# NoelShin/zutis

Measured on AMD Instinct MI355X. Metric: images/sec, COCO2017-val-shaped ViT-B/16 dense semantic segmentation @336px (ZUTIS forward + semantic predict), batches of 32 per GPU, 3 independent batches in flight, higher is better.
Workload: dtype f16x3 (fp32-class)

## Files before the change

### include/zutis_hip.h

```cpp
#ifndef ZUTIS_HIP_H
#define ZUTIS_HIP_H

#include <stddef.h>

#ifdef __cplusplus
extern "C" {
#endif

typedef struct ihipStream_t* zh_stream_t;

#define ZH_OK 0
#define ZH_ERR_ARG (-1)
#define ZH_ERR_HIP (-2)
#define ZH_ERR_WORKSPACE (-3)

#define ZH_ACT_NONE 0
#define ZH_ACT_QUICKGELU 1
#define ZH_ACT_RELU 2
#define ZH_ACT_SIGMOID 3
#define ZH_ACT_GELU_ERF 4

#define ZH_ABI_VERSION 245
int zh_version(void);
const char* zh_arch(void);
const char* zh_last_error(void);

int zh_dev_set_gemm_overrides(int group_m, int tile, int tile_small);

int zh_dev_gemm_plan(int mode, int M, int N, int K, int batch, long lda, long ldw, long ldc, long strideC, long planeC,
                     long ldr, long strideR, int res_rows, int out_kind, int act, int flags,
                     const void* C, const void* bias, const void* residual, int has_pos, int* plan);

int zh_dev_set_gemm_persist(int workgroups);

int zh_gemm_f16(const void* A, long lda, long strideA, const void* W, long ldw, long strideW,
                void* C, long ldc, long strideC, int out_f16,
                const float* bias, const float* residual, long ldr, long strideR, int res_rows,
                const void* pos_y, const void* pos_x, long ld_pos, int pos_h, int pos_w, int pos_f16,
                int act, int M, int N, int K, int batch, zh_stream_t stream);

int zh_gemm_f16_res16(const void* A, long lda, long strideA, const void* W, long ldw, long strideW,
                      void* C, long ldc, long strideC,
                      const float* bias, const void* residual, long ldr, long strideR, int res_rows,
                      int M, int N, int K, int batch, zh_stream_t stream);

#define ZH_GEMM_FIXED_K_ORDER 1
int zh_gemm_f16x3(const void* A, long lda, long strideA, long planeA, const void* W, long ldw, long strideW, long planeW,
                  void* C, long ldc, long strideC, long planeC, int out_kind, float out_scale,
                  const float* bias, const float* residual, long ldr, long strideR, int res_rows,
                  const void* pos_y, const void* pos_x, long ld_pos, int pos_h, int pos_w, int pos_f16,
                  int act, int M, int N, int K, int batch, int flags, zh_stream_t stream);

#define ZH_ATTN_QUERY_BLOCK 128
#define ZH_ATTN_KEY_TILE_F16 64
#define ZH_ATTN_KEY_TILE_X3 32
size_t zh_attention_splitk_workspace_size(int batch, int heads, int Tq, int head_dim, int ksplit);
int zh_attention_f16_splitk(const void* Q, long ldq, long strideQ, const void* K, long ldk, long strideK,
                            const void* V, long ldv, long strideV, void* O, long ldo, long strideO,
                            int batch, int heads, int Tq, int Tk, int head_dim, float scale,
                            long planeQ, long planeK, long planeV, long planeO, int ksplit, void* workspace, size_t workspace_bytes,
                            zh_stream_t stream);
int zh_attention_f16(const void* Q, long ldq, long strideQ, const void* K, long ldk, long strideK,
                     const void* V, long ldv, long strideV, void* O, long ldo, long strideO,
                     int batch, int heads, int Tq, int Tk, int head_dim, float scale,
                     long planeQ, long planeK, long planeV, long planeO, zh_stream_t stream);

int zh_attention_causal_f16(const void* Q, long ldq, long strideQ, const void* K, long ldk, long strideK,
                            const void* V, long ldv, long strideV, void* O, long ldo, long strideO,
                            int batch, int heads, int T, int head_dim, float scale,
                            long planeQ, long planeK, long planeV, long planeO, zh_stream_t stream);

int zh_dev_attention_plan(const void* Q, long ldq, long strideQ, const void* K, long ldk, long strideK,
                          const void* V, long ldv, long strideV, const void* O, long ldo, long strideO,
                          int batch, int heads, int Tq, int Tk, int head_dim, int causal,
                          long planeQ, long planeK, long planeV, long planeO, int ksplit, const void* workspace, size_t workspace_bytes,
                          int* plan);

int zh_embed_tokens_f32(const long long* tokens, const float* table, const float* pos, float* out, long n, int ctx, int D,
                        int vocab, zh_stream_t stream);
int zh_eot_rows_f32(const long long* tokens, const float* x, float* out, long n, int ctx, int D, zh_stream_t stream);
int zh_group_mean_l2norm(const float* x, float* out, int groups, int T, int E, zh_stream_t stream);

int zh_layernorm_f32(const float* x, long in_group_rows, long in_group_stride, long in_offset,
                     long out_group_rows, long out_group_stride, long out_offset,
                     const float* gamma, const float* beta, float eps,
                     float* out_f32, void* out_f16, void* out_f16_plus, float* out_f32_plus,
                     const float* add, int add_rows, int rows, int D, long lo_plane, int* status, zh_stream_t stream);
int zh_layernorm_f16(const void* x, long in_group_rows, long in_group_stride, long in_offset,
                     long out_group_rows, long out_group_stride, long out_offset,
                     const float* gamma, const float* beta, float eps,
                     float* out_f32, void* out_f16, void* out_f16_plus, float* out_f32_plus,
                     const float* add, int add_rows, int rows, int D, long lo_plane, int* status, zh_stream_t stream);
#define ZH_STATUS_RANGE 1
#define ZH_STATUS_NONFINITE 2
#define ZH_STATUS_LABEL 4

int zh_sum_layernorm_f32(const float* parts, int n_parts, long part_stride, const float* bias, const float* residual,
                         float* out_sum, const float* gamma, const float* beta, float eps,
                         float* out_f32, void* out_f16, long lo_plane,
                         long out_group_rows, long out_group_stride, long out_offset, int skip_first_in_group,
                         const float* gamma2, const float* beta2, float eps2, float* out2_f32, void* out2_f16, long lo_plane2,
                         long out2_group_rows, long out2_group_stride, long out2_offset,
                         int rows, int D, int* status, zh_stream_t stream);

int zh_assemble_tokens_ln(const float* patch_emb, const float* class_embedding, const float* pos_embed,
                          const float* gamma, const float* beta, float eps, float* out,
                          int B, int T, int D, zh_stream_t stream);

int zh_assemble_tokens_ln_f16(const float* patch_emb, const float* class_embedding, const float* pos_embed,
                              const float* gamma, const float* beta, float eps, void* out,
                              int B, int T, int D, zh_stream_t stream);

int zh_l2norm_rows(const float* x, float* out_f32, void* out_f16, float eps, int rows, int D, long lo_plane, float f16_scale, zh_stream_t stream);

size_t zh_global_ln_l2_workspace_size(int B, int M, int C);
int zh_global_ln_l2(const float* x, float* out_f32, void* out_f16, float eps, float l2_eps,
                    int B, int M, int C, void* workspace, size_t workspace_bytes, long lo_plane, float f16_scale, int* status,
                    zh_stream_t stream);

int zh_im2col_f16(const float* x, void* out, int B, int Cin, int H, int W, int patch, int Kpad, int pad_to_patch,
                  long lo_plane, zh_stream_t stream);

int zh_posembed_bicubic(const float* pos, float* out, int grid, int h, int w, int D, float scale_h, float scale_w,
                        int has_cls, zh_stream_t stream);

int zh_upsample2x_bilinear_cl(const float* x, float* out_f32, void* out_f16, int B, int h, int w, int D, long lo_plane,
                              int relu, zh_stream_t stream);

int zh_sine_pe(float* out, int h, int w, int D, float temperature, zh_stream_t stream);

int zh_add_rowperiodic_f16(const void* a, const float* add, void* out, long rows, int D, int add_rows, long a_lo_plane,
                           long lo_plane, zh_stream_t stream);

int zh_fill_f32(float* x, float value, long n, zh_stream_t stream);

int zh_cast_f32_f16(const float* x, const float* add, int add_rows, void* out, long rows, int D, long lo_plane, float f16_scale,
                    zh_stream_t stream);

int zh_upsample_argmax(const float* logits_lo, long long* labels, int B, int n, int h, int w, int H, int W,
                       float scale_h, float scale_w, zh_stream_t stream);

#define ZH_GT_U8 0
#define ZH_GT_RG16 1
int zh_upsample_argmax_score(const float* logits_lo, const unsigned char* gt, int gt_format, long long* hist_accum,
                             long long* labels, int B, int n, int h, int w, int H, int W, float scale_h, float scale_w,
                             zh_stream_t stream);

int zh_upsample_argmax_bytes(const float* logits_lo, unsigned char* labels_out, int label_format, unsigned char* overlay_out,
                             const unsigned char* packed, const int* desc, const unsigned char* palette, int alpha,
                             int B, int n, int h, int w, int H, int W, float scale_h, float scale_w, zh_stream_t stream);

int zh_upsample_bilinear_nchw(const float* x, float* out, unsigned char* mask_u8, float threshold, long planes,
                              int h, int w, int H, int W, float scale_h, float scale_w, zh_stream_t stream);

int zh_select_upsample_mask(const float* objectness, const float* masks, unsigned char* out_u8, long long* index, int B, int Q,
                            int h, int w, int H, int W, float scale_h, float scale_w, float threshold, zh_stream_t stream);

int zh_resize_nearest_u8(const unsigned char* x, unsigned char* out, int h, int w, int H, int W, float scale_h, float scale_w,
                         zh_stream_t stream);

int zh_confusion_hist(const long long* label_true, const long long* label_pred, long long* hist_accum, long total,
                      int n_class, zh_stream_t stream);

int zh_instance_mask_stats(const float* mask_proposals, long stride_image, float threshold, int B, int Q, int M,
                           float* sizes, float* confidence, unsigned char* binary, int* range_flag, zh_stream_t stream);
size_t zh_masked_mean_workspace_size(int B, int Q, int M, int E);
int zh_masked_mean_tokens(const float* tokens, const unsigned char* binary, const float* sizes, float* avg,
                          int B, int Q, int M, int E, void* workspace, size_t workspace_bytes, zh_stream_t stream);
int zh_instance_classify(const float* avg, const float* text, const float* confidence, float temperature,
                         int rows, int n_classes, int E, long long* category, float* score, zh_stream_t stream);
size_t zh_mask_iou_workspace_size(int n, long pixels);
int zh_mask_iou_counts(const unsigned char* masks, int n, long pixels, int* inter, int* uni,
                       void* workspace, size_t workspace_bytes, zh_stream_t stream);

#define ZH_RCN_KMAX 152
int zh_resize_crop_normalize_u8(const unsigned char* packed, long packed_bytes, const int* desc, int B, int n_px, int kmax,
                                const float* lut, float* out, zh_stream_t stream);
#define ZH_FILTER_BILINEAR 2
#define ZH_FILTER_BICUBIC 3
int zh_resize_normalize_u8(const unsigned char* packed, long packed_bytes, const int* desc, int B, int out_h, int out_w, int filter,
                           int kmax, const float* lut, float* out, zh_stream_t stream);

int zh_denormalize_u8(const float* x, unsigned char* rgb, int H, int W, const float* mean3, const float* std3,
                      zh_stream_t stream);
int zh_bgrid_coords(const unsigned char* rgb, int H, int W, double sigma_spatial, double sigma_luma, double sigma_chroma,
                    int* coords, zh_stream_t stream);
// ... 173 lines not shown
```

### zutis_amd/csrc/capi.hip

```cpp
#include "common.h"
#include <stdarg.h>

static thread_local char g_err[512] = "";

void zh_set_error(const char* fmt, ...) {
  va_list ap;
  va_start(ap, fmt);
  vsnprintf(g_err, sizeof(g_err), fmt, ap);
  va_end(ap);
}

extern "C" const char* zh_last_error(void) { return g_err; }
extern "C" int zh_version(void) { return ZH_ABI_VERSION; }
extern "C" const char* zh_arch(void) { return "gfx950"; }

#include <stdlib.h>
#include "gemm_dispatch.h"
static GemmDevOverrides& gemm_dev_state() {
  static GemmDevOverrides o = [] {
    GemmDevOverrides v{4, 0, 0};
    if (const char* g = getenv("ZH_GEMM_GROUP_M")) { const int x = atoi(g); if (x >= 1) v.group_m = x; }
    if (const char* t = getenv("ZH_GEMM_TILE")) v.tile = atoi(t);
    if (const char* t = getenv("ZH_GEMM_TILE_SMALL")) v.tile_small = atoi(t);
    return v;
  }();
  return o;
}
const GemmDevOverrides& gemm_dev_overrides() { return gemm_dev_state(); }
extern "C" int zh_dev_set_gemm_overrides(int group_m, int tile, int tile_small) {
  ZH_CHECK_ARG(group_m >= 0 && tile >= 0 && tile_small >= 0, "zh_dev_set_gemm_overrides: negative argument");
  GemmDevOverrides& o = gemm_dev_state();
  o.group_m = group_m >= 1 ? group_m : 4;
  o.tile = tile;
  o.tile_small = tile_small;
  return ZH_OK;
}

extern "C" int zh_dev_gemm_plan(int mode, int M, int N, int K, int batch, long lda, long ldw, long ldc, long strideC, long planeC,
                                long ldr, long strideR, int res_rows, int out_kind, int act, int flags,
                                const void* C, const void* bias, const void* residual, int has_pos, int* plan) {
  ZH_CHECK_ARG(plan && mode >= GEMM_F16 && mode <= GEMM_X2, "zh_dev_gemm_plan: null plan or mode %d not in {0 f16, 1 res16, 2 x3, 3 x2}", mode);
  ZH_CHECK_ARG(M > 0 && N > 0 && K > 0 && batch > 0, "zh_dev_gemm_plan: bad shape M=%d N=%d K=%d batch=%d", M, N, K, batch);
  const GemmProblem q = {mode, M, N, K, batch, lda, ldw, ldc, strideC, planeC, ldr, strideR, res_rows, out_kind, act, flags,
                         (uintptr_t)C, (uintptr_t)bias, (uintptr_t)residual, has_pos != 0, mode == GEMM_RES16};
  GemmPlan g;
  const int rc = mode <= GEMM_RES16 ? gemm_plan_f16(q, gemm_dev_overrides(), &g) : gemm_plan_x3(q, gemm_dev_overrides(), &g);
  if (rc != ZH_OK) return rc;
  const GemmTile* t = gemm_plan_tile(mode, g.code);
  ZH_CHECK_ARG(t || g.family == GEMM_SKINNY, "zh_dev_gemm_plan: the plan's tile code %d has no table row", g.code);
  plan[0] = g.family; plan[1] = g.code; plan[2] = t ? gemm_tile_m(*t) : 32; plan[3] = t ? gemm_tile_n(*t) : 32;
  plan[4] = g.path; plan[5] = (int)g.peel_rows;
  return ZH_OK;
}

#include "attention_dispatch.h"
extern "C" int zh_dev_attention_plan(const void* Q, long ldq, long strideQ, const void* K, long ldk, long strideK,
                                     const void* V, long ldv, long strideV, const void* O, long ldo, long strideO,
                                     int batch, int heads, int Tq, int Tk, int head_dim, int causal,
                                     long planeQ, long planeK, long planeV, long planeO, int ksplit, const void* workspace, size_t workspace_bytes,
                                     int* plan) {
  ZH_CHECK_ARG(plan, "zh_dev_attention_plan: null plan");
  AttnPlan a;
  const int rc = attn_plan(attn_problem(Q, ldq, strideQ, K, ldk, strideK, V, ldv, strideV, O, ldo, strideO, batch, heads, Tq, Tk, head_dim, causal,
                                        planeQ, planeK, planeV, planeO, ksplit, workspace, workspace_bytes), &a);
  if (rc != ZH_OK) return rc;
  ZH_CHECK_ARG(a.workspace_bytes <= 0x7FFFFFFF, "zh_dev_attention_plan: a workspace of %zu bytes does not fit the int row", a.workspace_bytes);
  plan[0] = a.variant; plan[1] = a.key_tile; plan[2] = a.nqb; plan[3] = (int)a.items; plan[4] = (int)a.grid; plan[5] = a.pipe;
  plan[6] = a.ksplit; plan[7] = a.kchunk; plan[8] = (int)a.workspace_bytes; plan[9] = (int)a.combine_grid;
  return ZH_OK;
}

static int gemm_persist_valid(int n) { return n >= 0 && n % 8 == 0; }
static int g_gemm_persist = [] {
  const char* e = getenv("ZH_GEMM_PERSIST");
  if (!e) return -1;
  char* end = nullptr;
  const long v = strtol(e, &end, 10);
  if (end == e || *end != 0 || v < 0 || v > (1 << 20) || !gemm_persist_valid((int)v)) {
    fprintf(stderr, "zutis_hip: ZH_GEMM_PERSIST=%s ignored (not 0 or a multiple of 8)\n", e);
    return -1;
  }
  return (int)v;
}();
int gemm_persist_cus() {
  if (g_gemm_persist >= 0) return g_gemm_persist;
  static const int auto_cus = [] {
    int dev = 0, cus = 0;
    if (hipGetDevice(&dev) != hipSuccess || hipDeviceGetAttribute(&cus, hipDeviceAttributeMultiprocessorCount, dev) != hipSuccess || cus < 8) return 256;
    return cus / 8 * 8;
  }();
  return auto_cus;
}
extern "C" int zh_dev_set_gemm_persist(int workgroups) {
  ZH_CHECK_ARG(workgroups >= -1 && (workgroups == -1 || gemm_persist_valid(workgroups)), "zh_dev_set_gemm_persist: %d is not -1 (auto), 0 (off) or a multiple of 8", workgroups);
  g_gemm_persist = workgroups;
  return ZH_OK;
}
```

### zutis_amd/csrc/gemm.hip

```cpp
#include "gemm_kernel.h"
#include "gemm_dispatch.h"

template <int WM, int WN, int TM, int TN, int STAGES, int VEC>
static bool launch_gemm(const GemmArgs& p, int batch, int out_f16, int res_f16, hipStream_t stream) {
  const int key = res_f16 * 16 + out_f16 * 8 + p.act;
  switch (key) {
    case 0 + ZH_ACT_NONE: launch_one<WM, WN, TM, TN, STAGES, 0, ZH_ACT_NONE, VEC, 0>(p, batch, stream); return true;
    case 0 + ZH_ACT_SIGMOID: launch_one<WM, WN, TM, TN, STAGES, 0, ZH_ACT_SIGMOID, VEC, 0>(p, batch, stream); return true;
    case 8 + ZH_ACT_NONE: launch_one<WM, WN, TM, TN, STAGES, 1, ZH_ACT_NONE, VEC, 0>(p, batch, stream); return true;
    case 8 + ZH_ACT_QUICKGELU: launch_one<WM, WN, TM, TN, STAGES, 1, ZH_ACT_QUICKGELU, VEC, 0>(p, batch, stream); return true;
    case 8 + ZH_ACT_RELU: launch_one<WM, WN, TM, TN, STAGES, 1, ZH_ACT_RELU, VEC, 0>(p, batch, stream); return true;
    case 8 + ZH_ACT_GELU_ERF: launch_one<WM, WN, TM, TN, STAGES, 1, ZH_ACT_GELU_ERF, VEC, 0>(p, batch, stream); return true;
    case 16 + 8 + ZH_ACT_NONE: launch_one<WM, WN, TM, TN, STAGES, 3, ZH_ACT_NONE, VEC, 0>(p, batch, stream); return true;
    default: return false;
  }
}

static int gemm_f16_impl(const void* A, long lda, long strideA, const void* W, long ldw, long strideW,
                         void* C, long ldc, long strideC, int out_f16,
                         const float* bias, const void* residual, int res_f16, long ldr, long strideR, int res_rows,
                         const void* pos_y, const void* pos_x, long ld_pos, int pos_h, int pos_w, int pos_f16,
                         int act, int M, int N, int K, int batch, hipStream_t stream) {
  GemmArgs p;
  GemmProblem q;
  GemmPlan plan;
  int rc = gemm_prepare("zh_gemm_f16", res_f16 ? GEMM_RES16 : GEMM_F16, A, lda, strideA, 0, W, ldw, strideW, 0, C, ldc, strideC, 0, out_f16 ? 1 : 0, 1.0f,
                        bias, residual, ldr, strideR, res_rows, pos_y, pos_x, ld_pos, pos_h, pos_w, pos_f16, act, M, N, K, batch, 0, &p, &q);
  if (rc != ZH_OK) return rc;
  ZH_CHECK_ARG(!res_f16 || (out_f16 && act == ZH_ACT_NONE), "zh_gemm_f16_res16: an fp16 residual goes with an fp16 output and no activation");
  if ((rc = gemm_plan_f16(q, gemm_dev_overrides(), &plan)) != ZH_OK) return rc;
  if (plan.peel_rows)
    return gemm_tail_peel(plan.peel_rows, M, A, lda, C, ldc, out_f16 ? 2 : 4, residual, ldr, res_f16 ? 2 : 4, res_rows,
                          [&](const void* a, void* c, const void* r, int rows, int m) {
                            return gemm_f16_impl(a, lda, strideA, W, ldw, strideW, c, ldc, strideC, out_f16, bias, r, res_f16, ldr, strideR, rows,
                                                 pos_y, pos_x, ld_pos, pos_h, pos_w, pos_f16, act, m, N, K, 1, stream);
                          });
  const int ok = gemm_launch_plan<GEMM_TILES_F16>(plan, [&](auto row) {
    constexpr GemmTile t = decltype(row)::t;
    return launch_gemm<t.wm, t.wn, t.tm, t.tn, t.stages, decltype(row)::vec>(p, batch, out_f16, res_f16, stream);
  }, std::make_index_sequence<std::size(GEMM_TILES_F16)>{});
  ZH_CHECK_ARG(ok >= 0, "zh_gemm_f16: the plan's tile code %d has no table row", plan.code);
  ZH_CHECK_ARG(ok, "zh_gemm_f16: (out_f16=%d, act=%d) is not an instantiated epilogue (f32: none|sigmoid; f16: none|quickgelu|relu|gelu_erf)",
               out_f16, act);
  ZH_CHECK_LAUNCH("zh_gemm_f16");
  return ZH_OK;
}

extern "C" int zh_gemm_f16(const void* A, long lda, long strideA, const void* W, long ldw, long strideW,
                           void* C, long ldc, long strideC, int out_f16,
                           const float* bias, const float* residual, long ldr, long strideR, int res_rows,
                           const void* pos_y, const void* pos_x, long ld_pos, int pos_h, int pos_w, int pos_f16,
                           int act, int M, int N, int K, int batch, hipStream_t stream) {
  return gemm_f16_impl(A, lda, strideA, W, ldw, strideW, C, ldc, strideC, out_f16, bias, residual, 0, ldr, strideR, res_rows,
                       pos_y, pos_x, ld_pos, pos_h, pos_w, pos_f16, act, M, N, K, batch, stream);
}

extern "C" int zh_gemm_f16_res16(const void* A, long lda, long strideA, const void* W, long ldw, long strideW,
                                 void* C, long ldc, long strideC,
                                 const float* bias, const void* residual, long ldr, long strideR, int res_rows,
                                 int M, int N, int K, int batch, hipStream_t stream) {
  ZH_CHECK_ARG(residual, "zh_gemm_f16_res16: null residual (zh_gemm_f16 is the form without one)");
  return gemm_f16_impl(A, lda, strideA, W, ldw, strideW, C, ldc, strideC, 1, bias, residual, 1, ldr, strideR, res_rows,
                       nullptr, nullptr, 0, 0, 0, 0, ZH_ACT_NONE, M, N, K, batch, stream);
}
```

### zutis_amd/csrc/gemm_dispatch.h

```cpp
#pragma once
#include "common.h"
#include <utility>
#ifndef RING64
#define RING64 6
#endif
#ifndef ZH_SKINNY_MAX_ROWS
#define ZH_SKINNY_MAX_ROWS 128
#endif
#ifndef ZH_SKINNY_MAX_BLOCKS
#define ZH_SKINNY_MAX_BLOCKS 512
#endif

struct GemmDevOverrides { int group_m; int tile; int tile_small; };
const GemmDevOverrides& gemm_dev_overrides();

enum { GEMM_F16 = 0, GEMM_RES16 = 1, GEMM_X3 = 2, GEMM_X2 = 3 };
enum { GEMM_RING = 0, GEMM_SKINNY = 1 };
enum { GEMM_STORE_SCALAR = 0, GEMM_STORE_DIRECT = 1, GEMM_STORE_WIDE = 2 };

struct GemmProblem {
  int mode, M, N, K, batch; long lda, ldw, ldc, strideC, planeC, ldr, strideR; int res_rows, out_kind, act, flags;
  uintptr_t C, bias, residual; bool has_pos, res_f16;
};
struct GemmPlan { int family, code, path; long peel_rows; };

struct GemmTile { int code, wm, wn, tm, tn, stages; };
constexpr GemmTile GEMM_TILES_F16[] = {
  {128, 2, 2, 4, 4, 4},
  {64, 2, 2, 4, 2, 4},
  {192, 2, 4, 8, 3, 4},
  {256, 2, 4, 8, 4, 4},
  {2128, 2, 2, 4, 4, 8},
  {2064, 2, 2, 4, 2, 8},
  {3064, 2, 2, 2, 2, 8},
  {7032, 2, 2, 2, 2, 7},
  {7096, 2, 2, 4, 3, 5},
  {7128, 2, 2, 4, 4, 5},
};
constexpr GemmTile GEMM_TILES_X3[] = {
  {64, 2, 2, 4, 2, 3},
  {512, 2, 4, 8, 4, 2},
  {448, 2, 4, 6, 4, 2},
  {256, 4, 2, 4, 4, 3},
  {192, 4, 2, 3, 4, 3},
  {96, 4, 2, 2, 3, 3},
  {3064, 2, 2, 2, 2, 4},
  {3066, 2, 2, 2, 2, RING64},
  {1288, 4, 2, 2, 4, 4},
  {6496, 4, 2, 2, 3, 2},
  {6464, 4, 2, 2, 2, 3},
  {7096, 4, 2, 2, 3, 4},
  {7128, 4, 2, 2, 4, 3},
};
constexpr GemmTile GEMM_TILES_X2[] = {
  {64, 2, 2, 4, 2, 3},
  {512, 4, 2, 4, 8, 3},
  {5122, 2, 4, 8, 4, 2},
  {5124, 2, 4, 8, 4, 3},
  {4484, 4, 2, 3, 8, 3},
  {448, 2, 4, 6, 4, 3},
  {256, 4, 2, 4, 4, 3},
  {192, 4, 2, 3, 4, 4},
  {96, 4, 2, 2, 3, 3},
  {3064, 2, 2, 2, 2, 4},
  {3066, 2, 2, 2, 2, RING64},
  {6464, 4, 2, 2, 2, 3},
  {1288, 4, 2, 2, 4, 4},
  {6496, 4, 2, 2, 3, 2},
};
constexpr int gemm_tile_m(const GemmTile& t) { return t.wm * t.tm * 16; }
constexpr int gemm_tile_n(const GemmTile& t) { return t.wn * t.tn * 16; }
template <size_t R>
constexpr const GemmTile* gemm_tile(const GemmTile (&rows)[R], int code) {
  for (size_t i = 0; i < R; ++i) if (rows[i].code == code) return &rows[i];
  return nullptr;
}
static inline const GemmTile* gemm_plan_tile(int mode, int code) {
  if (mode <= GEMM_RES16) return code ? gemm_tile(GEMM_TILES_F16, code) : GEMM_TILES_F16;
  if (mode == GEMM_X3) return code ? gemm_tile(GEMM_TILES_X3, code) : GEMM_TILES_X3;
  return code ? gemm_tile(GEMM_TILES_X2, code) : GEMM_TILES_X2;
}
template <const auto& ROWS, size_t I, int VEC> struct GemmRow { static constexpr GemmTile t = ROWS[I]; static constexpr int vec = VEC; };
template <const auto& ROWS, class L, size_t... I>
static inline int gemm_launch_plan(const GemmPlan& plan, L&& launch, std::index_sequence<I...>) {
  if (plan.path != GEMM_STORE_WIDE) return plan.path == GEMM_STORE_SCALAR ? launch(GemmRow<ROWS, 0, 0>{}) : launch(GemmRow<ROWS, 0, 1>{});
  int ok = -1;
  (void)((ROWS[I].code == plan.code && ((ok = launch(GemmRow<ROWS, I, 2>{})), true)) || ...);
  return ok;
}

static inline bool gemm_vec_ok(const GemmProblem& q) {
  const int esz = q.out_kind == 0 ? 4 : 2;
  return q.N % 4 == 0 && q.ldc % 4 == 0 && q.strideC % 4 == 0 && (q.C & (4 * esz - 1)) == 0 && (!q.bias || (q.bias & 15) == 0) &&
         (!q.residual || (q.ldr % 4 == 0 && q.strideR % 4 == 0 && (q.residual & (q.res_f16 ? 7 : 15)) == 0));
}
static inline bool gemm_wide_ok(const GemmProblem& q) {
  const int esz = q.out_kind == 0 ? 4 : 2;
  if (!(gemm_vec_ok(q) && (q.C & 15) == 0 && (q.ldc * esz) % 16 == 0 && (q.strideC * esz) % 16 == 0 && (q.N * esz) % 16 == 0)) return false;
  if (q.mode <= GEMM_RES16)
    return !q.residual || (q.res_f16 ? (q.ldr % 8 == 0 && q.strideR % 8 == 0 && (q.residual & 15) == 0) : q.out_kind == 0);
  return (q.out_kind != 1 || !q.residual) && (q.out_kind != 2 || q.planeC % 8 == 0);
}

static inline bool zh_pos_tables_ok(const void* pos_y, const void* pos_x, long ld_pos, int pos_h, int pos_w, int N) {
  if (!pos_y && !pos_x) return true;
  return pos_y && pos_x && pos_h > 0 && pos_w > 0 && ld_pos >= N && ld_pos % 8 == 0 && N % 4 == 0 &&
         (((uintptr_t)pos_y | (uintptr_t)pos_x) & 15) == 0;
}

template <class Args>
static inline int gemm_prepare(const char* fn, int mode, const void* A, long lda, long strideA, long planeA, const void* W, long ldw, long strideW,
                               long planeW, void* C, long ldc, long strideC, long planeC, int out_kind, float out_scale, const float* bias,
                               const void* residual, long ldr, long strideR, int res_rows, const void* pos_y, const void* pos_x, long ld_pos,
                               int pos_h, int pos_w, int pos_f16, int act, int M, int N, int K, int batch, int flags, Args* pp, GemmProblem* q) {
  ZH_CHECK_ARG(A && W && C, "%s: null operand", fn);
  ZH_CHECK_ARG(M > 0 && N > 0 && K > 0 && batch > 0, "%s: bad shape M=%d N=%d K=%d batch=%d", fn, M, N, K, batch);
  ZH_CHECK_ARG(K % 64 == 0, "%s: K=%d must be a multiple of 64", fn, K);
  ZH_CHECK_ARG(lda % 8 == 0 && ldw % 8 == 0 && strideA % 8 == 0 && strideW % 8 == 0 && planeA % 8 == 0 && planeW % 8 == 0,
               "%s: lda/ldw/strides/planes must be multiples of 8 halves (16-byte rows)", fn);
  ZH_CHECK_ARG(((uintptr_t)A & 15) == 0 && ((uintptr_t)W & 15) == 0, "%s: A/W must be 16-byte aligned", fn);
  ZH_CHECK_ARG(act >= 0 && act <= 4, "%s: bad activation %d", fn, act);
  ZH_CHECK_ARG((long)(M - 1) * lda + K <= 0xFFFFFFFFL && (long)(N - 1) * ldw + K <= 0xFFFFFFFFL,
               "%s: an operand exceeds 2^32 elements per batch item (M=%d lda=%ld N=%d ldw=%ld)", fn, M, lda, N, ldw);
  ZH_CHECK_ARG(!residual || res_rows > 0, "%s: residual needs res_rows > 0", fn);
  ZH_CHECK_ARG(zh_pos_tables_ok(pos_y, pos_x, ld_pos, pos_h, pos_w, N), "%s: pos tables need both pointers 16-byte aligned, "
               "pos_h, pos_w > 0, ld_pos %% 8 == 0 and N %% 4 == 0", fn);
  *q = {mode, M, N, K, batch, lda, ldw, ldc, strideC, planeC, ldr, strideR, res_rows, out_kind, act, flags,
        (uintptr_t)C, (uintptr_t)bias, (uintptr_t)residual, pos_y != nullptr, mode == GEMM_RES16};
  Args& p = *pp;
  p.A = (const half_t*)A; p.lda = lda; p.sA = strideA; p.planeA = planeA;
  p.W = (const half_t*)W; p.ldw = ldw; p.sW = strideW; p.planeW = planeW;
  p.C = C; p.ldc = ldc; p.sC = strideC; p.planeC = planeC; p.out_scale = out_scale;
  p.bias = bias; p.R = (const float*)residual; p.ldr = ldr; p.sR = strideR; p.res_rows = res_rows;
  p.pos_y = pos_y; p.pos_x = pos_x; p.ld_pos = ld_pos; p.pos_hw = pos_h * pos_w; p.pos_w = pos_w; p.pos_f16 = pos_f16;
  p.M = M; p.N = N; p.K = K; p.act = act; p.nbm = p.nbn = 0;
  p.group_m = gemm_dev_overrides().group_m;
  p.vec_ok = gemm_vec_ok(*q);
  return ZH_OK;
}

static inline double tiling_cost(long M, long N, int batch, int BM, int BN, int bpc, double eff) {
  const long tiles = (long)zh_cdiv(M, BM) * zh_cdiv(N, BN) * batch;
  const long slots = 256L * bpc;
  const long rounds = (tiles + slots - 1) / slots;
  return (double)rounds * BM * BN * bpc / eff;
}
static inline long gemm_tiles(const GemmProblem& q, int BM, int BN) { return (long)zh_cdiv(q.M, BM) * zh_cdiv(q.N, BN) * q.batch; }

static inline long gemm_peel_rows(const GemmProblem& q, const GemmTile& big, bool wide) {
  if (!wide || q.batch != 1 || q.has_pos || (q.residual && q.res_rows < q.M)) return 0;
  const long BM = gemm_tile_m(big), nbm = zh_cdiv(q.M, BM), nbn = zh_cdiv(q.N, gemm_tile_n(big)), tiles = nbm * nbn, rem = tiles % 256;
  if (tiles <= 4 * 256 || rem == 0 || rem > 64) return 0;
  const long r = (rem + nbn - 1) / nbn;
  return r * nbn <= 64 ? (nbm - r) * BM : 0;
}
template <class Call>
static inline int gemm_tail_peel(long M1, int M, const void* A, long lda, void* C, long ldc, int c_esz, const void* residual, long ldr,
                                 int r_esz, int res_rows, Call&& call) {
  const int rc = call(A, C, residual, residual ? res_rows : 0, (int)M1);
  if (rc != ZH_OK) return rc;
  return call((const char*)A + M1 * lda * 2, (char*)C + M1 * ldc * c_esz, residual ? (const char*)residual + M1 * ldr * r_esz : nullptr,
              residual ? (int)(res_rows - M1) : 0, (int)(M - M1));
}

static inline GemmPlan gemm_ring_plan(const GemmProblem& q, int pick, bool wide, long peel_rows) {
  return {GEMM_RING, wide ? pick : 0, wide ? GEMM_STORE_WIDE : (gemm_vec_ok(q) ? GEMM_STORE_DIRECT : GEMM_STORE_SCALAR), peel_rows};
}

static inline int gemm_plan_f16(const GemmProblem& q, const GemmDevOverrides& ov, GemmPlan* plan) {
  const int M = q.M, N = q.N, batch = q.batch;
  ZH_CHECK_ARG(gemm_tiles(q, 64, 64) < (1L << 31), "zh_gemm_f16: grid too large");
  const int forced = ov.tile ? ov.tile : (M <= 4096 ? ov.tile_small : 0);
  ZH_CHECK_ARG(!forced || gemm_tile(GEMM_TILES_F16, forced),
               "zh_gemm_f16: ZH_GEMM_TILE(_SMALL)=%d is not a tile code (64|128|192|256|2064|2128|3064|7032|7096|7128)", forced);
  const double c256 = tiling_cost(M, N, batch, 256, 256, 1, 1.0);
  const double c192 = tiling_cost(M, N, batch, 256, 192, 1, 0.95);
  const double c128 = tiling_cost(M, N, batch, 128, 128, 2, 0.8);
  int pick = (c128 < c256 && c128 < c192) ? 128 : (c192 < c256 ? 192 : 256);
  const long t128 = gemm_tiles(q, 128, 128);
  if (t128 <= 96) pick = 3064;
  else if (pick == 128 && t128 <= 256 && N <= 768) pick = 64;
  if (pick == 3064) pick = 7032;
  else if ((pick == 64 || pick == 128) && N % 96 == 0 && (long)zh_cdiv(M, 128) * (N / 96) * batch <= 256) pick = 7096;
  else if (pick == 128 && t128 <= 256) pick = 7128;
  if (forced) pick = forced;
  const bool wide = gemm_wide_ok(q);
  const long peel = ((pick == 256 || pick == 192) && !forced) ? gemm_peel_rows(q, *gemm_plan_tile(q.mode, pick), wide) : 0;
  *plan = gemm_ring_plan(q, pick, wide, peel);
  return ZH_OK;
}

static inline int gemm_plan_x3(const GemmProblem& q, const GemmDevOverrides& ov, GemmPlan* plan) {
  const int M = q.M, N = q.N, batch = q.batch;
  const bool x2 = q.mode == GEMM_X2;
  ZH_CHECK_ARG(gemm_tiles(q, 64, 64) < (1L << 31), "zh_gemm_f16x3: grid too large");
  const int forced = ov.tile;
  const bool own = forced && (x2 ? gemm_tile(GEMM_TILES_X2, forced) != nullptr
                                 : gemm_tile(GEMM_TILES_X3, forced) && !((forced == 7096 || forced == 7128) && q.has_pos));
  const int max_rows = forced == 32 ? (1 << 30) : ((forced || (q.flags & ZH_GEMM_FIXED_K_ORDER)) ? 0 : ZH_SKINNY_MAX_ROWS);
  const long sk_blocks = gemm_tiles(q, 32, 32);
  if (!q.has_pos && M <= max_rows && sk_blocks <= 65535L * 8 && (forced == 32 || sk_blocks <= ZH_SKINNY_MAX_BLOCKS)) {
    *plan = {GEMM_SKINNY, 32, gemm_vec_ok(q) ? 1 : 0, 0};
    return ZH_OK;
  }
  const double c256 = tiling_cost(M, N, batch, 256, 128, 1, 1.0);
  const double c192 = tiling_cost(M, N, batch, 192, 128, 1, 0.95);
  const double c64 = tiling_cost(M, N, batch, 128, 64, 2, 0.7);
  int pick = (c64 < c256 && c64 < c192) ? 64 : (c192 < c256 ? 192 : 256);
  if (M >= 4096) {
    const double cbig = tiling_cost(M, N, batch, 256, 256, 1, 1.25);
    const double c448 = tiling_cost(M, N, batch, 192, 256, 1, 1.2);
    const double cur = pick == 64 ? c64 : (pick == 192 ? c192 : c256);
    if (cbig < cur && cbig <= c448) pick = 512;
    else if (c448 < cur) pick = 448;
  }
  const long t64 = gemm_tiles(q, 128, 64);
  if (pick == 64 && M <= 4096 && N % 96 == 0 && t64 > 256 && (long)zh_cdiv(M, 128) * (N / 96) * batch <= 256) pick = 96;
  if (pick == 64 && gemm_tiles(q, 64, 64) <= 256) pick = 3064;
  if (pick == 64 && t64 <= 256) pick = 6464;
  if (own) pick = forced;
  if (pick == 64 && gemm_tiles(q, 128, 128) <= 256 && t64 > 256) pick = 1288;
  if (pick == 96 && !forced && !x2 && !q.has_pos) pick = 7096;
  if ((pick == 512 || pick == 448 || pick == 5122 || pick == 5124 || pick == 4484) &&
      ((long)(M - 1) * q.lda + q.K > 0x7FFFFFFFL || (long)(N - 1) * q.ldw + q.K > 0x7FFFFFFFL)) pick = 256;
  const bool wide = gemm_wide_ok(q);
  const long peel = ((pick == 512 || pick == 448) && !forced && ov.tile_small == 0) ? gemm_peel_rows(q, *gemm_plan_tile(q.mode, pick), wide) : 0;
  *plan = gemm_ring_plan(q, pick, wide, peel);
  return ZH_OK;
}
```

### zutis_amd/csrc/gemm_x3.hip

```cpp
#include "gemm_kernel.h"
#include "gemm_skinny.h"
#include "gemm_dispatch.h"

template <int WM, int WN, int TM, int TN, int STAGES, int VEC, int SP = 1>
static bool launch_x3(const GemmArgs& p, int batch, int out_kind, hipStream_t stream) {
  const int key = out_kind * 8 + p.act;
  switch (key) {
    case 0 + ZH_ACT_NONE: launch_one<WM, WN, TM, TN, STAGES, 0, ZH_ACT_NONE, VEC, SP>(p, batch, stream); return true;
    case 0 + ZH_ACT_SIGMOID: launch_one<WM, WN, TM, TN, STAGES, 0, ZH_ACT_SIGMOID, VEC, SP>(p, batch, stream); return true;
    case 8 + ZH_ACT_NONE: launch_one<WM, WN, TM, TN, STAGES, 1, ZH_ACT_NONE, VEC, SP>(p, batch, stream); return true;
    case 16 + ZH_ACT_NONE: launch_one<WM, WN, TM, TN, STAGES, 2, ZH_ACT_NONE, VEC, SP>(p, batch, stream); return true;
    default: break;
  }
  if (VEC == 2) {
    switch (key) {
      case 8 + ZH_ACT_QUICKGELU: launch_one<WM, WN, TM, TN, STAGES, 1, ZH_ACT_QUICKGELU, 2, SP>(p, batch, stream); return true;
      case 8 + ZH_ACT_RELU: launch_one<WM, WN, TM, TN, STAGES, 1, ZH_ACT_RELU, 2, SP>(p, batch, stream); return true;
      case 8 + ZH_ACT_GELU_ERF: launch_one<WM, WN, TM, TN, STAGES, 1, ZH_ACT_GELU_ERF, 2, SP>(p, batch, stream); return true;
      case 16 + ZH_ACT_QUICKGELU: launch_one<WM, WN, TM, TN, STAGES, 2, ZH_ACT_QUICKGELU, 2, SP>(p, batch, stream); return true;
      case 16 + ZH_ACT_RELU: launch_one<WM, WN, TM, TN, STAGES, 2, ZH_ACT_RELU, 2, SP>(p, batch, stream); return true;
      case 16 + ZH_ACT_GELU_ERF: launch_one<WM, WN, TM, TN, STAGES, 2, ZH_ACT_GELU_ERF, 2, SP>(p, batch, stream); return true;
      default: break;
    }
  }
  return false;
}

template <const auto& ROWS, int SP>
static int launch_x3_plan(const GemmPlan& plan, const GemmArgs& p, int batch, int out_kind, hipStream_t stream) {
  return gemm_launch_plan<ROWS>(plan, [&](auto row) {
    constexpr GemmTile t = decltype(row)::t;
    return launch_x3<t.wm, t.wn, t.tm, t.tn, t.stages, decltype(row)::vec, SP>(p, batch, out_kind, stream);
  }, std::make_index_sequence<std::size(ROWS)>{});
}

extern "C" int zh_gemm_f16x3(const void* A, long lda, long strideA, long planeA, const void* W, long ldw, long strideW, long planeW,
                             void* C, long ldc, long strideC, long planeC, int out_kind, float out_scale,
                             const float* bias, const float* residual, long ldr, long strideR, int res_rows,
                             const void* pos_y, const void* pos_x, long ld_pos, int pos_h, int pos_w, int pos_f16,
                             int act, int M, int N, int K, int batch, int flags, hipStream_t stream) {
  const bool x2 = planeW == 0;
  GemmArgs p;
  GemmProblem q;
  GemmPlan plan;
  int rc = gemm_prepare("zh_gemm_f16x3", x2 ? GEMM_X2 : GEMM_X3, A, lda, strideA, planeA, W, ldw, strideW, planeW, C, ldc, strideC, planeC, out_kind, out_scale,
                        bias, residual, ldr, strideR, res_rows, pos_y, pos_x, ld_pos, pos_h, pos_w, pos_f16, act, M, N, K, batch, flags, &p, &q);
  if (rc != ZH_OK) return rc;
  ZH_CHECK_ARG(planeA != 0, "zh_gemm_f16x3: A must be a split pair (plane offset of the lo half)");
  ZH_CHECK_ARG(out_kind >= 0 && out_kind <= 2, "zh_gemm_f16x3: out_kind %d not in {0 f32, 1 f16, 2 split pair}", out_kind);
  ZH_CHECK_ARG(out_kind != 2 || (planeC != 0 && planeC % 4 == 0), "zh_gemm_f16x3: split output needs planeC (multiple of 4)");
  ZH_CHECK_ARG(!residual || out_kind == 0 || act == ZH_ACT_NONE, "zh_gemm_f16x3: a residual of an fp16 / split output goes with no activation");
  ZH_CHECK_ARG(out_scale > 0.0f, "zh_gemm_f16x3: out_scale must be positive");
  if ((rc = gemm_plan_x3(q, gemm_dev_overrides(), &plan)) != ZH_OK) return rc;
  if (plan.peel_rows)
    return gemm_tail_peel(plan.peel_rows, M, A, lda, C, ldc, out_kind == 0 ? 4 : 2, residual, ldr, 4, res_rows,
                          [&](const void* a, void* c, const void* r, int rows, int m) {
                            return zh_gemm_f16x3(a, lda, strideA, planeA, W, ldw, strideW, planeW, c, ldc, strideC, planeC, out_kind, out_scale, bias,
                                                 (const float*)r, ldr, strideR, rows, pos_y, pos_x, ld_pos, pos_h, pos_w, pos_f16, act, m, N, K, 1, flags, stream);
                          });
  int ok = 1;
  if (plan.family == GEMM_SKINNY) {
    if (x2) launch_skinny<1>(p, batch, out_kind, stream);
    else launch_skinny<2>(p, batch, out_kind, stream);
  } else
    ok = x2 ? launch_x3_plan<GEMM_TILES_X2, 2>(plan, p, batch, out_kind, stream) : launch_x3_plan<GEMM_TILES_X3, 1>(plan, p, batch, out_kind, stream);
  ZH_CHECK_ARG(ok >= 0, "zh_gemm_f16x3: the plan's tile code %d has no table row", plan.code);
  ZH_CHECK_ARG(ok, "zh_gemm_f16x3: (out_kind=%d, act=%d) is not an instantiated epilogue", out_kind, act);
  ZH_CHECK_LAUNCH("zh_gemm_f16x3");
  return ZH_OK;
}
```

### zutis_amd/csrc/plan.hip

```cpp
#include "common.h"
#include <string.h>

struct ZhCmd { int op; int pad; unsigned long long a[32]; };

static inline float zh_w2f(unsigned long long w) { unsigned u = (unsigned)w; float f; memcpy(&f, &u, 4); return f; }
static inline double zh_w2d(unsigned long long w) { double d; memcpy(&d, &w, 8); return d; }

static int zh_dispatch(const ZhCmd& c, zh_stream_t stream) {
  switch (c.op) {
#define ZH_PLAN_CASES
#include "plan_gen.inc"
#undef ZH_PLAN_CASES
    default: zh_set_error("zh_plan_run: unknown op %d", c.op); return ZH_ERR_ARG;
  }
}

static const char* const zh_plan_names[] = {
#define ZH_PLAN_NAMES
#include "plan_gen.inc"
#undef ZH_PLAN_NAMES
};

extern "C" const char* zh_plan_op_name(int op) {
  const int n = (int)(sizeof(zh_plan_names) / sizeof(zh_plan_names[0]));
  return (op >= 0 && op < n) ? zh_plan_names[op] : nullptr;
}

extern "C" int zh_plan_run(const void* cmds, int n, zh_stream_t stream) {
  const ZhCmd* c = (const ZhCmd*)cmds;
  for (int i = 0; i < n; ++i) {
    const int rc = zh_dispatch(c[i], stream);
    if (rc != ZH_OK) return rc;
  }
  return ZH_OK;
}

extern "C" int zh_plan_run2(const void* cmds_a, int na, zh_stream_t stream_a, const void* cmds_b, int nb, zh_stream_t stream_b) {
  const ZhCmd* a = (const ZhCmd*)cmds_a;
  const ZhCmd* b = (const ZhCmd*)cmds_b;
  for (int i = 0; i < na || i < nb; ++i) {
    if (i < na) { const int rc = zh_dispatch(a[i], stream_a); if (rc != ZH_OK) return rc; }
    if (i < nb) { const int rc = zh_dispatch(b[i], stream_b); if (rc != ZH_OK) return rc; }
  }
  return ZH_OK;
}

extern "C" int zh_plan_run_multi(const void* const* cmds, const int* n, const zh_stream_t* streams, int count) {
  ZH_CHECK_ARG(cmds && n && streams && count > 0, "zh_plan_run_multi: bad arguments");
  int longest = 0;
  for (int j = 0; j < count; ++j) longest = n[j] > longest ? n[j] : longest;
  for (int i = 0; i < longest; ++i)
    for (int j = 0; j < count; ++j)
      if (i < n[j]) { const int rc = zh_dispatch(((const ZhCmd*)cmds[j])[i], streams[j]); if (rc != ZH_OK) return rc; }
  return ZH_OK;
}
```

Before: 3041.

## Make GEMM tile planning account for concurrent streams in flight

Adds a thread-local in-flight count, set by the multi-stream plan runners, that the GEMM tile planner uses to scale tile counts when estimating wave quantization and picking tiles and tail peeling. With several independent batches sharing the GPU, larger tiles can fill the CUs without being penalized for partial rounds. A fallback keeps the single-stream plan when the concurrent pick has a smaller tile area or an unwanted two-slot tile. The risk is that the assumed overlap does not happen, which would leave individual GEMMs under-filling the machine.

```diff
diff --git a/include/zutis_hip.h b/include/zutis_hip.h
--- a/include/zutis_hip.h
+++ b/include/zutis_hip.h
@@ -20,7 +20,7 @@
 #define ZH_ACT_SIGMOID 3
 #define ZH_ACT_GELU_ERF 4
 
-#define ZH_ABI_VERSION 245
+#define ZH_ABI_VERSION 246
 int zh_version(void);
 const char* zh_arch(void);
 const char* zh_last_error(void);
@@ -32,6 +32,11 @@
                      const void* C, const void* bias, const void* residual, int has_pos, int* plan);
 
 int zh_dev_set_gemm_persist(int workgroups);
+
+int zh_dev_set_gemm_inflight(int inflight);
+int zh_dev_gemm_plan_inflight(int mode, int M, int N, int K, int batch, long lda, long ldw, long ldc, long strideC, long planeC,
+                              long ldr, long strideR, int res_rows, int out_kind, int act, int flags,
+                              const void* C, const void* bias, const void* residual, int has_pos, int inflight, int* plan);
 
 int zh_gemm_f16(const void* A, long lda, long strideA, const void* W, long ldw, long strideW,
                 void* C, long ldc, long strideC, int out_f16,
diff --git a/zutis_amd/csrc/capi.hip b/zutis_amd/csrc/capi.hip
--- a/zutis_amd/csrc/capi.hip
+++ b/zutis_amd/csrc/capi.hip
@@ -36,15 +36,33 @@
   return ZH_OK;
 }
 
+static thread_local int t_gemm_inflight = 1;
+static int g_gemm_inflight_forced = 0;
+int gemm_inflight() { return g_gemm_inflight_forced ? g_gemm_inflight_forced : t_gemm_inflight; }
+GemmInflightScope::GemmInflightScope(int n) : prev(t_gemm_inflight) { t_gemm_inflight = n < 1 ? 1 : (n > ZH_GEMM_INFLIGHT_MAX ? ZH_GEMM_INFLIGHT_MAX : n); }
+GemmInflightScope::~GemmInflightScope() { t_gemm_inflight = prev; }
+extern "C" int zh_dev_set_gemm_inflight(int inflight) {
+  ZH_CHECK_ARG(inflight >= 0 && inflight <= ZH_GEMM_INFLIGHT_MAX, "zh_dev_set_gemm_inflight: %d is not 0 (not forced) or 1 .. %d", inflight, ZH_GEMM_INFLIGHT_MAX);
+  g_gemm_inflight_forced = inflight;
+  return ZH_OK;
+}
+
 extern "C" int zh_dev_gemm_plan(int mode, int M, int N, int K, int batch, long lda, long ldw, long ldc, long strideC, long planeC,
                                 long ldr, long strideR, int res_rows, int out_kind, int act, int flags,
                                 const void* C, const void* bias, const void* residual, int has_pos, int* plan) {
+  return zh_dev_gemm_plan_inflight(mode, M, N, K, batch, lda, ldw, ldc, strideC, planeC, ldr, strideR, res_rows, out_kind, act, flags, C, bias, residual,
+                                   has_pos, gemm_inflight(), plan);
+}
+extern "C" int zh_dev_gemm_plan_inflight(int mode, int M, int N, int K, int batch, long lda, long ldw, long ldc, long strideC, long planeC,
+                                         long ldr, long strideR, int res_rows, int out_kind, int act, int flags,
+                                         const void* C, const void* bias, const void* residual, int has_pos, int inflight, int* plan) {
   ZH_CHECK_ARG(plan && mode >= GEMM_F16 && mode <= GEMM_X2, "zh_dev_gemm_plan: null plan or mode %d not in {0 f16, 1 res16, 2 x3, 3 x2}", mode);
   ZH_CHECK_ARG(M > 0 && N > 0 && K > 0 && batch > 0, "zh_dev_gemm_plan: bad shape M=%d N=%d K=%d batch=%d", M, N, K, batch);
+  ZH_CHECK_ARG(inflight >= 1 && inflight <= ZH_GEMM_INFLIGHT_MAX, "zh_dev_gemm_plan_inflight: inflight %d not in 1 .. %d", inflight, ZH_GEMM_INFLIGHT_MAX);
   const GemmProblem q = {mode, M, N, K, batch, lda, ldw, ldc, strideC, planeC, ldr, strideR, res_rows, out_kind, act, flags,
                          (uintptr_t)C, (uintptr_t)bias, (uintptr_t)residual, has_pos != 0, mode == GEMM_RES16};
   GemmPlan g;
-  const int rc = mode <= GEMM_RES16 ? gemm_plan_f16(q, gemm_dev_overrides(), &g) : gemm_plan_x3(q, gemm_dev_overrides(), &g);
+  const int rc = mode <= GEMM_RES16 ? gemm_plan_f16(q, gemm_dev_overrides(), &g, inflight) : gemm_plan_x3(q, gemm_dev_overrides(), &g, inflight);
   if (rc != ZH_OK) return rc;
   const GemmTile* t = gemm_plan_tile(mode, g.code);
   ZH_CHECK_ARG(t || g.family == GEMM_SKINNY, "zh_dev_gemm_plan: the plan's tile code %d has no table row", g.code);
diff --git a/zutis_amd/csrc/gemm.hip b/zutis_amd/csrc/gemm.hip
--- a/zutis_amd/csrc/gemm.hip
+++ b/zutis_amd/csrc/gemm.hip
@@ -28,7 +28,7 @@
                         bias, residual, ldr, strideR, res_rows, pos_y, pos_x, ld_pos, pos_h, pos_w, pos_f16, act, M, N, K, batch, 0, &p, &q);
   if (rc != ZH_OK) return rc;
   ZH_CHECK_ARG(!res_f16 || (out_f16 && act == ZH_ACT_NONE), "zh_gemm_f16_res16: an fp16 residual goes with an fp16 output and no activation");
-  if ((rc = gemm_plan_f16(q, gemm_dev_overrides(), &plan)) != ZH_OK) return rc;
+  if ((rc = gemm_plan_f16(q, gemm_dev_overrides(), &plan, gemm_inflight())) != ZH_OK) return rc;
   if (plan.peel_rows)
     return gemm_tail_peel(plan.peel_rows, M, A, lda, C, ldc, out_f16 ? 2 : 4, residual, ldr, res_f16 ? 2 : 4, res_rows,
                           [&](const void* a, void* c, const void* r, int rows, int m) {
diff --git a/zutis_amd/csrc/gemm_dispatch.h b/zutis_amd/csrc/gemm_dispatch.h
--- a/zutis_amd/csrc/gemm_dispatch.h
+++ b/zutis_amd/csrc/gemm_dispatch.h
@@ -13,6 +13,19 @@
 
 struct GemmDevOverrides { int group_m; int tile; int tile_small; };
 const GemmDevOverrides& gemm_dev_overrides();
+
+int gemm_inflight();
+struct GemmInflightScope {
+  int prev;
+  explicit GemmInflightScope(int n);
+  ~GemmInflightScope();
+  GemmInflightScope(const GemmInflightScope&) = delete;
+  GemmInflightScope& operator=(const GemmInflightScope&) = delete;
+};
+#ifndef ZH_GEMM_INFLIGHT_MIN_ROWS
+#define ZH_GEMM_INFLIGHT_MIN_ROWS 2048
+#endif
+#define ZH_GEMM_INFLIGHT_MAX 64
 
 enum { GEMM_F16 = 0, GEMM_RES16 = 1, GEMM_X3 = 2, GEMM_X2 = 3 };
 enum { GEMM_RING = 0, GEMM_SKINNY = 1 };
@@ -139,20 +152,25 @@
   return ZH_OK;
 }
 
-static inline double tiling_cost(long M, long N, int batch, int BM, int BN, int bpc, double eff) {
-  const long tiles = (long)zh_cdiv(M, BM) * zh_cdiv(N, BN) * batch;
+static inline double tiling_cost(long M, long N, int batch, int BM, int BN, int bpc, double eff, int inflight = 1) {
+  const long tiles = (long)zh_cdiv(M, BM) * zh_cdiv(N, BN) * batch * inflight;
   const long slots = 256L * bpc;
   const long rounds = (tiles + slots - 1) / slots;
   return (double)rounds * BM * BN * bpc / eff;
 }
 static inline long gemm_tiles(const GemmProblem& q, int BM, int BN) { return (long)zh_cdiv(q.M, BM) * zh_cdiv(q.N, BN) * q.batch; }
-
-static inline long gemm_peel_rows(const GemmProblem& q, const GemmTile& big, bool wide) {
+static inline int gemm_inflight_counted(const GemmProblem& q, int inflight) {
+  if (inflight <= 1 || q.M < ZH_GEMM_INFLIGHT_MIN_ROWS || gemm_tiles(q, 128, 64) <= 256) return 1;
+  return inflight < ZH_GEMM_INFLIGHT_MAX ? inflight : ZH_GEMM_INFLIGHT_MAX;
+}
+
+static inline long gemm_peel_rows(const GemmProblem& q, const GemmTile& big, bool wide, int inflight = 1) {
   if (!wide || q.batch != 1 || q.has_pos || (q.residual && q.res_rows < q.M)) return 0;
-  const long BM = gemm_tile_m(big), nbm = zh_cdiv(q.M, BM), nbn = zh_cdiv(q.N, gemm_tile_n(big)), tiles = nbm * nbn, rem = tiles % 256;
+  const long BM = gemm_tile_m(big), nbm = zh_cdiv(q.M, BM), nbn = zh_cdiv(q.N, gemm_tile_n(big)), tiles = nbm * nbn * inflight, rem = tiles % 256;
   if (tiles <= 4 * 256 || rem == 0 || rem > 64) return 0;
-  const long r = (rem + nbn - 1) / nbn;
-  return r * nbn <= 64 ? (nbm - r) * BM : 0;
+  const long per = (rem + inflight - 1) / inflight;
+  const long r = (per + nbn - 1) / nbn;
+  return (r * nbn * inflight <= 64 && r < nbm) ? (nbm - r) * BM : 0;
 }
 template <class Call>
 static inline int gemm_tail_peel(long M1, int M, const void* A, long lda, void* C, long ldc, int c_esz, const void* residual, long ldr,
@@ -167,30 +185,30 @@
   return {GEMM_RING, wide ? pick : 0, wide ? GEMM_STORE_WIDE : (gemm_vec_ok(q) ? GEMM_STORE_DIRECT : GEMM_STORE_SCALAR), peel_rows};
 }
 
-static inline int gemm_plan_f16(const GemmProblem& q, const GemmDevOverrides& ov, GemmPlan* plan) {
+static inline int gemm_plan_f16_counted(const GemmProblem& q, const GemmDevOverrides& ov, GemmPlan* plan, int fl) {
   const int M = q.M, N = q.N, batch = q.batch;
   ZH_CHECK_ARG(gemm_tiles(q, 64, 64) < (1L << 31), "zh_gemm_f16: grid too large");
   const int forced = ov.tile ? ov.tile : (M <= 4096 ? ov.tile_small : 0);
   ZH_CHECK_ARG(!forced || gemm_tile(GEMM_TILES_F16, forced),
                "zh_gemm_f16: ZH_GEMM_TILE(_SMALL)=%d is not a tile code (64|128|192|256|2064|2128|3064|7032|7096|7128)", forced);
-  const double c256 = tiling_cost(M, N, batch, 256, 256, 1, 1.0);
-  const double c192 = tiling_cost(M, N, batch, 256, 192, 1, 0.95);
-  const double c128 = tiling_cost(M, N, batch, 128, 128, 2, 0.8);
+  const double c256 = tiling_cost(M, N, batch, 256, 256, 1, 1.0, fl);
+  const double c192 = tiling_cost(M, N, batch, 256, 192, 1, 0.95, fl);
+  const double c128 = tiling_cost(M, N, batch, 128, 128, 2, 0.8, fl);
   int pick = (c128 < c256 && c128 < c192) ? 128 : (c192 < c256 ? 192 : 256);
-  const long t128 = gemm_tiles(q, 128, 128);
+  const long t128 = fl * gemm_tiles(q, 128, 128);
   if (t128 <= 96) pick = 3064;
   else if (pick == 128 && t128 <= 256 && N <= 768) pick = 64;
   if (pick == 3064) pick = 7032;
-  else if ((pick == 64 || pick == 128) && N % 96 == 0 && (long)zh_cdiv(M, 128) * (N / 96) * batch <= 256) pick = 7096;
+  else if ((pick == 64 || pick == 128) && N % 96 == 0 && fl * (long)zh_cdiv(M, 128) * (N / 96) * batch <= 256) pick = 7096;
   else if (pick == 128 && t128 <= 256) pick = 7128;
   if (forced) pick = forced;
   const bool wide = gemm_wide_ok(q);
-  const long peel = ((pick == 256 || pick == 192) && !forced) ? gemm_peel_rows(q, *gemm_plan_tile(q.mode, pick), wide) : 0;
+  const long peel = ((pick == 256 || pick == 192) && !forced) ? gemm_peel_rows(q, *gemm_plan_tile(q.mode, pick), wide, fl) : 0;
   *plan = gemm_ring_plan(q, pick, wide, peel);
   return ZH_OK;
 }
 
-static inline int gemm_plan_x3(const GemmProblem& q, const GemmDevOverrides& ov, GemmPlan* plan) {
+static inline int gemm_plan_x3_counted(const GemmProblem& q, const GemmDevOverrides& ov, GemmPlan* plan, int fl) {
   const int M = q.M, N = q.N, batch = q.batch;
   const bool x2 = q.mode == GEMM_X2;
   ZH_CHECK_ARG(gemm_tiles(q, 64, 64) < (1L << 31), "zh_gemm_f16x3: grid too large");
@@ -203,28 +221,53 @@
     *plan = {GEMM_SKINNY, 32, gemm_vec_ok(q) ? 1 : 0, 0};
     return ZH_OK;
   }
-  const double c256 = tiling_cost(M, N, batch, 256, 128, 1, 1.0);
-  const double c192 = tiling_cost(M, N, batch, 192, 128, 1, 0.95);
-  const double c64 = tiling_cost(M, N, batch, 128, 64, 2, 0.7);
+  const double c256 = tiling_cost(M, N, batch, 256, 128, 1, 1.0, fl);
+  const double c192 = tiling_cost(M, N, batch, 192, 128, 1, 0.95, fl);
+  const double c64 = tiling_cost(M, N, batch, 128, 64, 2, 0.7, fl);
   int pick = (c64 < c256 && c64 < c192) ? 64 : (c192 < c256 ? 192 : 256);
   if (M >= 4096) {
-    const double cbig = tiling_cost(M, N, batch, 256, 256, 1, 1.25);
-    const double c448 = tiling_cost(M, N, batch, 192, 256, 1, 1.2);
+    const double cbig = tiling_cost(M, N, batch, 256, 256, 1, 1.25, fl);
+    const double c448 = tiling_cost(M, N, batch, 192, 256, 1, 1.2, fl);
     const double cur = pick == 64 ? c64 : (pick == 192 ? c192 : c256);
     if (cbig < cur && cbig <= c448) pick = 512;
     else if (c448 < cur) pick = 448;
   }
-  const long t64 = gemm_tiles(q, 128, 64);
-  if (pick == 64 && M <= 4096 && N % 96 == 0 && t64 > 256 && (long)zh_cdiv(M, 128) * (N / 96) * batch <= 256) pick = 96;
-  if (pick == 64 && gemm_tiles(q, 64, 64) <= 256) pick = 3064;
+  const long t64 = fl * gemm_tiles(q, 128, 64);
+  if (pick == 64 && M <= 4096 && N % 96 == 0 && t64 > 256 && fl * (long)zh_cdiv(M, 128) * (N / 96) * batch <= 256) pick = 96;
+  if (pick == 64 && fl * gemm_tiles(q, 64, 64) <= 256) pick = 3064;
   if (pick == 64 && t64 <= 256) pick = 6464;
   if (own) pick = forced;
-  if (pick == 64 && gemm_tiles(q, 128, 128) <= 256 && t64 > 256) pick = 1288;
+  if (pick == 64 && fl * gemm_tiles(q, 128, 128) <= 256 && t64 > 256) pick = 1288;
   if (pick == 96 && !forced && !x2 && !q.has_pos) pick = 7096;
   if ((pick == 512 || pick == 448 || pick == 5122 || pick == 5124 || pick == 4484) &&
       ((long)(M - 1) * q.lda + q.K > 0x7FFFFFFFL || (long)(N - 1) * q.ldw + q.K > 0x7FFFFFFFL)) pick = 256;
   const bool wide = gemm_wide_ok(q);
-  const long peel = ((pick == 512 || pick == 448) && !forced && ov.tile_small == 0) ? gemm_peel_rows(q, *gemm_plan_tile(q.mode, pick), wide) : 0;
+  const long peel = ((pick == 512 || pick == 448) && !forced && ov.tile_small == 0) ? gemm_peel_rows(q, *gemm_plan_tile(q.mode, pick), wide, fl) : 0;
   *plan = gemm_ring_plan(q, pick, wide, peel);
   return ZH_OK;
 }
+
+static inline long gemm_plan_area(int mode, const GemmPlan& p) {
+  const GemmTile* t = p.family == GEMM_RING ? gemm_plan_tile(mode, p.code) : nullptr;
+  return t ? (long)gemm_tile_m(*t) * gemm_tile_n(*t) : 32L * 32;
+}
+static inline bool gemm_two_slot(int mode, const GemmPlan& p) {
+  return mode >= GEMM_X3 && p.family == GEMM_RING && (p.code == 512 || p.code == 448);
+}
+template <class PlanFn>
+static inline int gemm_plan_in_flight(const GemmProblem& q, const GemmDevOverrides& ov, GemmPlan* plan, int fl, PlanFn&& counted) {
+  int rc = counted(q, ov, plan, fl);
+  if (rc != ZH_OK || fl == 1) return rc;
+  GemmPlan lone;
+  if ((rc = counted(q, ov, &lone, 1)) != ZH_OK) return rc;
+  if (gemm_plan_area(q.mode, *plan) < gemm_plan_area(q.mode, lone)) *plan = lone;
+  else if (gemm_two_slot(q.mode, *plan) && !gemm_two_slot(q.mode, lone) && !(q.K >= 1024 && fl >= 3)) *plan = lone;
+  return ZH_OK;
+}
+static inline int gemm_plan_f16(const GemmProblem& q, const GemmDevOverrides& ov, GemmPlan* plan, int inflight = 1) {
+  const int fl = (inflight >= 3 && q.N <= 768) ? gemm_inflight_counted(q, inflight) : 1;
+  return gemm_plan_in_flight(q, ov, plan, fl, gemm_plan_f16_counted);
+}
+static inline int gemm_plan_x3(const GemmProblem& q, const GemmDevOverrides& ov, GemmPlan* plan, int inflight = 1) {
+  return gemm_plan_in_flight(q, ov, plan, gemm_inflight_counted(q, inflight), gemm_plan_x3_counted);
+}
diff --git a/zutis_amd/csrc/gemm_x3.hip b/zutis_amd/csrc/gemm_x3.hip
--- a/zutis_amd/csrc/gemm_x3.hip
+++ b/zutis_amd/csrc/gemm_x3.hip
@@ -51,7 +51,7 @@
   ZH_CHECK_ARG(out_kind != 2 || (planeC != 0 && planeC % 4 == 0), "zh_gemm_f16x3: split output needs planeC (multiple of 4)");
   ZH_CHECK_ARG(!residual || out_kind == 0 || act == ZH_ACT_NONE, "zh_gemm_f16x3: a residual of an fp16 / split output goes with no activation");
   ZH_CHECK_ARG(out_scale > 0.0f, "zh_gemm_f16x3: out_scale must be positive");
-  if ((rc = gemm_plan_x3(q, gemm_dev_overrides(), &plan)) != ZH_OK) return rc;
+  if ((rc = gemm_plan_x3(q, gemm_dev_overrides(), &plan, gemm_inflight())) != ZH_OK) return rc;
   if (plan.peel_rows)
     return gemm_tail_peel(plan.peel_rows, M, A, lda, C, ldc, out_kind == 0 ? 4 : 2, residual, ldr, 4, res_rows,
                           [&](const void* a, void* c, const void* r, int rows, int m) {
diff --git a/zutis_amd/csrc/plan.hip b/zutis_amd/csrc/plan.hip
--- a/zutis_amd/csrc/plan.hip
+++ b/zutis_amd/csrc/plan.hip
@@ -1,4 +1,5 @@
 #include "common.h"
+#include "gemm_dispatch.h"
 #include <string.h>
 
 struct ZhCmd { int op; int pad; unsigned long long a[32]; };
@@ -38,6 +39,7 @@
 extern "C" int zh_plan_run2(const void* cmds_a, int na, zh_stream_t stream_a, const void* cmds_b, int nb, zh_stream_t stream_b) {
   const ZhCmd* a = (const ZhCmd*)cmds_a;
   const ZhCmd* b = (const ZhCmd*)cmds_b;
+  const GemmInflightScope inflight(2);
   for (int i = 0; i < na || i < nb; ++i) {
     if (i < na) { const int rc = zh_dispatch(a[i], stream_a); if (rc != ZH_OK) return rc; }
     if (i < nb) { const int rc = zh_dispatch(b[i], stream_b); if (rc != ZH_OK) return rc; }
@@ -49,6 +51,7 @@
   ZH_CHECK_ARG(cmds && n && streams && count > 0, "zh_plan_run_multi: bad arguments");
   int longest = 0;
   for (int j = 0; j < count; ++j) longest = n[j] > longest ? n[j] : longest;
+  const GemmInflightScope inflight(count);
   for (int i = 0; i < longest; ++i)
     for (int j = 0; j < count; ++j)
       if (i < n[j]) { const int rc = zh_dispatch(((const ZhCmd*)cmds[j])[i], streams[j]); if (rc != ZH_OK) return rc; }
```

New measurement: 3084, median of 6. +1.4%, better.
